# Arthur151/ROMP

Measured on NVIDIA H100. Metric: frames/sec 512x512 ROMP-HRNet32 (whole hot path), higher is better.
Workload: dtype bf16

## Files before the change

### romp_b200/csrc/conv_block_tc.cu

```cuda
#include "conv_tc.cuh"
#include "tc_device.cuh"

namespace b200romp {

namespace {

constexpr int kBlkThreads = 384;
constexpr int kRowB = 128;
constexpr int kHaloW = 12, kHaloH = 20;
constexpr int kTapBytes = 64 * kRowB;
constexpr int kWBytes = 9 * kTapBytes;
constexpr int kStagePayload = kHaloH * kHaloW * kRowB;
constexpr int kStageBytes = (282 * kRowB + 1023) / 1024 * 1024;
constexpr int kMidBytes = 256 * kRowB;
constexpr int kSmemBytes = 2 * kWBytes + kStageBytes + kMidBytes + 1024  + 1024 ;
static_assert(kSmemBytes <= 227 * 1024, "fused block does not fit shared memory");

template <bool FOLD>
__device__ __forceinline__ constexpr bool blk_skip(int tap, int k) {
  return FOLD && ((tap % 3 == 0 && k < 2) || (tap % 3 == 2 && k >= 2));
}

__device__ __forceinline__ void consumers_bar_sync() { asm volatile("bar.sync 1, 256;" ::: "memory"); }

__device__ __forceinline__ uint32_t ld_shared_b32(uint32_t addr) {
  uint32_t v;
  asm volatile("ld.shared.b32 %0, [%1];" : "=r"(v) : "r"(addr));
  return v;
}
__device__ __forceinline__ void st_shared_b32(uint32_t addr, uint32_t v) {
  asm volatile("st.shared.b32 [%0], %1;" ::"r"(addr), "r"(v) : "memory");
}
template <typename T>
__device__ __forceinline__ T opaque(T v) {
  uint64_t u = (uint64_t)v;
  asm volatile("mov.b64 %0, %0;" : "+l"(u));
  return (T)u;
}
__device__ __forceinline__ uint32_t pack_bf16x2(float a, float b) {
  const __nv_bfloat162 v = __floats2bfloat162_rn(a, b);
  return *reinterpret_cast<const uint32_t*>(&v);
}

}

template <bool FOLD>
__global__ void __launch_bounds__(kBlkThreads, 1)
conv_block_tc_kernel(const __grid_constant__ CUtensorMap tmap, const ConvParams p, const uint8_t* __restrict__ w1pack,
                     const uint8_t* __restrict__ w2pack, const float* __restrict__ bias1, int tiles_x, int tiles_y, int num_tiles) {
  extern __shared__ uint8_t smem_raw[];
  uint8_t* smem = reinterpret_cast<uint8_t*>((reinterpret_cast<uintptr_t>(smem_raw) + 1023) & ~(uintptr_t)1023);
  uint8_t* sW1 = smem;
  uint8_t* sW2 = smem + kWBytes;
  uint8_t* sA = smem + 2 * kWBytes;
  uint8_t* sMid = sA + kStageBytes;
  uint64_t* full = reinterpret_cast<uint64_t*>(sMid + kMidBytes);
  uint64_t* empty = full + 1;
  uint64_t* w_full = full + 2;

  const int warp = threadIdx.x >> 5;
  if (threadIdx.x == 0) {
    mbar_init(full, 1);
    mbar_init(empty, 256);
    mbar_init(w_full, 1);
    fence_barrier_init();
  }
  __syncthreads();
  pdl_trigger();
  const int per_frame = tiles_x * tiles_y;

  if (warp == 0) {
    if (elect_one()) {
      mbar_arrive_expect_tx(w_full, 2 * kWBytes);
      for (int t = 0; t < 9; ++t) {
        bulk_copy_g2s(sW1 + t * kTapBytes, w1pack + (size_t)t * kTapBytes, kTapBytes, w_full);
        bulk_copy_g2s(sW2 + t * kTapBytes, w2pack + (size_t)t * kTapBytes, kTapBytes, w_full);
      }
      pdl_wait();
      const uint64_t pol = l2_policy_stream();
      uint32_t phase = 0;
      for (int tile = blockIdx.x; tile < num_tiles; tile += gridDim.x, phase ^= 1) {
        const int n = tile / per_frame, rem = tile % per_frame;
        const int y0 = (rem / tiles_x) * 16, x0 = (rem % tiles_x) * 8;
        mbar_wait(empty, phase ^ 1);
        mbar_arrive_expect_tx(full, kStagePayload);
        tma_load_4d(sA, &tmap, full, 0, x0 - 2, y0 - 2, n, pol);
      }
    }
  } else if (warp >= 4) {
    const int g = (warp >> 2) - 1, t = threadIdx.x & 127, w = t >> 5, l = t & 31;
    pdl_wait();
    mbar_wait(w_full, 0);
    const int cl = 2 * (l & 3);
    uint32_t phase = 0;
    for (int tile = blockIdx.x; tile < num_tiles; tile += gridDim.x, phase ^= 1) {
      const uint32_t w1_base = opaque(smem_u32(sW1)), w2_base = opaque(smem_u32(sW2)), a_base = opaque(smem_u32(sA)),
                     mid_base = opaque(smem_u32(sMid));
      const float* b1p = opaque(bias1);
      const float* b2p = opaque(p.bias);
      const int n = tile / per_frame, rem = tile % per_frame;
      const int y0 = (rem / tiles_x) * 16, x0 = (rem % tiles_x) * 8;
      mbar_wait(full, phase);

      float acc[2][32];
#pragma unroll
      for (int h = 0; h < 2; ++h)
#pragma unroll
        for (int j = 0; j < 32; ++j) acc[h][j] = 0.f;
      uint32_t scale_d = 0;
      wgmma_fence();
#pragma unroll
      for (int tap = 0; tap < 9; ++tap) {
        const uint32_t a_tap = a_base + (uint32_t)((128 * g + (tap / 3) * kHaloW + tap % 3) * kRowB);
        const uint32_t b_tap = w1_base + (uint32_t)(tap * kTapBytes);
#pragma unroll
        for (int k = 0; k < 4; ++k) {
          if (blk_skip<FOLD>(tap, k)) continue;
          const uint64_t bdesc = make_smem_desc(b_tap + k * 32, 8 * kRowB, kSw128);
          wgmma_n64(acc[0], make_smem_desc(a_tap + k * 32, 8 * kRowB, kSw128), bdesc, scale_d, false);
          wgmma_n64(acc[1], make_smem_desc(a_tap + 64 * kRowB + k * 32, 8 * kRowB, kSw128), bdesc, scale_d, false);
          scale_d = 1;
        }
      }
      wgmma_commit();
      uint32_t rv[2][8];
#pragma unroll
      for (int e = 0; e < 2; ++e) {
        const int hr = (8 * g + 2 * w + e + 2) * kHaloW + (l >> 2) + 2;
#pragma unroll
        for (int j = 0; j < 8; ++j) rv[e][j] = ld_shared_b32(a_base + hr * kRowB + ((j ^ (hr & 7)) << 4) + 2 * cl);
      }
      wgmma_wait<0>();
      mbar_arrive(empty);

      consumers_bar_sync();
#pragma unroll
      for (int h = 0; h < 2; ++h) {
#pragma unroll
        for (int e = 0; e < 2; ++e) {
          const int m = 64 * (2 * g + h) + 16 * w + (l >> 2) + 8 * e;
          const int my = m / kHaloW, mx = m % kHaloW;
          const bool inside = my < 18 && mx < 10 && (unsigned)(y0 - 1 + my) < (unsigned)p.Hout && (unsigned)(x0 - 1 + mx) < (unsigned)p.Wout;
          const uint32_t row = mid_base + m * kRowB;
#pragma unroll
          for (int j = 0; j < 8; ++j) {
            const int c = 8 * j + cl;
            float a = fmaxf(acc[h][4 * j + 2 * e] + __ldg(b1p + c), 0.f);
            float b = fmaxf(acc[h][4 * j + 2 * e + 1] + __ldg(b1p + c + 1), 0.f);
            if (!inside) a = b = 0.f;
            st_shared_b32(row + ((j ^ (m & 7)) << 4) + 2 * cl, pack_bf16x2(a, b));
          }
        }
      }
      fence_proxy_async();
      consumers_bar_sync();

      float acc2[32];
#pragma unroll
      for (int j = 0; j < 32; ++j) acc2[j] = 0.f;
      scale_d = 0;
      wgmma_fence();
#pragma unroll
      for (int tap = 0; tap < 9; ++tap) {
        const uint32_t a_tap = mid_base + (uint32_t)(((8 * g + tap / 3) * kHaloW + tap % 3) * kRowB);
        const uint32_t b_tap = w2_base + (uint32_t)(tap * kTapBytes);
#pragma unroll
        for (int k = 0; k < 4; ++k) {
          if (blk_skip<FOLD>(tap, k)) continue;
          wgmma_n64(acc2, make_smem_desc(a_tap + k * 32, kHaloW * kRowB, kSw128), make_smem_desc(b_tap + k * 32, 8 * kRowB, kSw128),
                    scale_d, false);
          scale_d = 1;
        }
      }
      wgmma_commit();
      wgmma_wait<0>();

      __nv_bfloat16* out = reinterpret_cast<__nv_bfloat16*>(p.out);
#pragma unroll
      for (int e = 0; e < 2; ++e) {
        const size_t pix = ((size_t)n * p.Hout + y0 + 8 * g + 2 * w + e) * p.Wout + x0 + (l >> 2);
        __nv_bfloat162* o = reinterpret_cast<__nv_bfloat162*>(out + pix * p.out_C + p.out_c_off + cl);
#pragma unroll
        for (int j = 0; j < 8; ++j) {
          const int c = 8 * j + cl;
          float a = acc2[4 * j + 2 * e] + __ldg(b2p + c), b = acc2[4 * j + 2 * e + 1] + __ldg(b2p + c + 1);
          const float2 r = res_pair(rv[e][j]);
          a += r.x; b += r.y;
          o[4 * j] = __floats2bfloat162_rn(fmaxf(a, 0.f), fmaxf(b, 0.f));
        }
      }
    }
  }
}

bool tc_block_supported(const ConvParams& p) {
  if (p.in_dtype != B200ROMP_BF16 || p.out_dtype != B200ROMP_BF16 || p.res_dtype != B200ROMP_BF16) return false;
  if (p.cin != 64 || p.cout != 64 || p.up != 1 || p.out_nchw || p.pow_channel >= 0 || p.input_norm || !p.relu) return false;
  if (p.Hin != p.Hout || p.Win != p.Wout || p.Hout % 16 != 0 || p.Wout % 8 != 0) return false;
  if (p.in_C % 8 != 0 || p.in_c_off % 8 != 0 || p.out_C % 8 != 0 || p.out_c_off % 8 != 0) return false;
  if (p.res != p.in || p.res_C != p.in_C || p.res_c_off != p.in_c_off || p.res_broadcast) return false;
  return (reinterpret_cast<uintptr_t>(p.in) & 15) == 0;
}

int tc_block_prepare(const ConvParams& p, const float* w1_oihw, const float* b1, const float* w2_oihw, int sm_count,
                     TcConvPlan* plan, std::vector<void*>* allocs) {
  PFN_encodeTiled encode = tc_get_encode();
  if (!encode) {
    set_error("conv_block_tc: cuTensorMapEncodeTiled is unavailable");
    return B200ROMP_ECUDA;
  }
  plan->kind = 60;
  plan->eb = 2;
  plan->cin = plan->cout = plan->nt = 64;
  plan->grid_x = sm_count;
  plan->grid_y = 1;
  plan->stages = 1;
  plan->smem_bytes = kSmemBytes;
  int rc = tc_pack_weights(w1_oihw, 64, 64, 9, 64, &plan->d_wpack, allocs, kRowB, 2);
  if (rc) return rc;
  rc = tc_pack_weights(w2_oihw, 64, 64, 9, 64, &plan->d_wpack2, allocs, kRowB, 2);
  if (rc) return rc;
  void* db1 = nullptr;
  B2R_CUDA_OK(cudaMalloc(&db1, 64 * sizeof(float)));
  allocs->push_back(db1);
  B2R_CUDA_OK(cudaMemcpy(db1, b1, 64 * sizeof(float), cudaMemcpyHostToDevice));
  plan->d_bias1 = static_cast<const float*>(db1);
  CUtensorMap tm;
  const cuuint64_t gdim[4] = {64, (cuuint64_t)p.Win, (cuuint64_t)p.Hin, (cuuint64_t)p.B};
  const cuuint64_t gstr[3] = {(cuuint64_t)p.in_C * 2, (cuuint64_t)p.Win * p.in_C * 2, (cuuint64_t)p.Hin * p.Win * p.in_C * 2};
  const cuuint32_t box[4] = {64, kHaloW, kHaloH, 1};
  const cuuint32_t estr[4] = {1, 1, 1, 1};
  void* base = const_cast<uint8_t*>(static_cast<const uint8_t*>(p.in) + (size_t)p.in_c_off * 2);
  CUresult cr = encode(&tm, CU_TENSOR_MAP_DATA_TYPE_BFLOAT16, 4, base, gdim, gstr, box, estr, CU_TENSOR_MAP_INTERLEAVE_NONE,
                       CU_TENSOR_MAP_SWIZZLE_128B, CU_TENSOR_MAP_L2_PROMOTION_L2_128B, CU_TENSOR_MAP_FLOAT_OOB_FILL_NONE);
  if (cr != CUDA_SUCCESS) {
    set_error("conv_block_tc: cuTensorMapEncodeTiled failed with %d", (int)cr);
    return B200ROMP_ECUDA;
  }
  memcpy(plan->tmap_in, &tm, sizeof(tm));
  B2R_CUDA_OK(cudaFuncSetAttribute(conv_block_tc_kernel<false>, cudaFuncAttributeMaxDynamicSharedMemorySize, kSmemBytes));
  B2R_CUDA_OK(cudaFuncSetAttribute(conv_block_tc_kernel<true>, cudaFuncAttributeMaxDynamicSharedMemorySize, kSmemBytes));
  return B200ROMP_OK;
}

int tc_block_launch(const TcConvPlan& plan, const ConvParams& p, cudaStream_t stream) {
  CUtensorMap tm;
  memcpy(&tm, plan.tmap_in, sizeof(tm));
  const int tiles_x = p.Wout / 8, tiles_y = p.Hout / 16;
  const int num_tiles = tiles_x * tiles_y * p.B;
  const dim3 grid(std::min(plan.grid_x, num_tiles));
  auto kern = plan.fold ? conv_block_tc_kernel<true> : conv_block_tc_kernel<false>;
  B2R_CUDA_OK(tc_launch(kern, grid, kBlkThreads, plan.smem_bytes, stream, tm, p, reinterpret_cast<const uint8_t*>(plan.d_wpack),
                        reinterpret_cast<const uint8_t*>(plan.d_wpack2), plan.d_bias1, tiles_x, tiles_y, num_tiles));
  return B200ROMP_OK;
}

}
```

Baseline: 3221.

## Ping-pong two consumer warpgroups over double-buffered tiles in fused residual block

Restructures the fused conv-conv residual block so each consumer warpgroup owns a whole tile in its own double-buffered smem slot, and the two warpgroups alternate issuing their wgmma phases through 'issued' mbarriers. The conv1 output is written back into the input slot instead of a separate mid buffer. Producer and consumer register budgets are rebalanced with setmaxnreg, and bias values are hoisted into registers once per CTA. The aim is to overlap one warpgroup's epilogue with the other's tensor-core work and to take the TMA load off the critical path. The cost is higher register pressure (two conv1 accumulator sets per thread) and more complex barrier phase logic.

Result: faster. 3274 (median of 6 runs) (+1.6%).

```diff
diff --git a/romp_b200/csrc/conv_block_tc.cu b/romp_b200/csrc/conv_block_tc.cu
--- a/romp_b200/csrc/conv_block_tc.cu
+++ b/romp_b200/csrc/conv_block_tc.cu
@@ -10,18 +10,26 @@
 constexpr int kHaloW = 12, kHaloH = 20;
 constexpr int kTapBytes = 64 * kRowB;
 constexpr int kWBytes = 9 * kTapBytes;
-constexpr int kStagePayload = kHaloH * kHaloW * kRowB;
-constexpr int kStageBytes = (282 * kRowB + 1023) / 1024 * 1024;
-constexpr int kMidBytes = 256 * kRowB;
-constexpr int kSmemBytes = 2 * kWBytes + kStageBytes + kMidBytes + 1024  + 1024 ;
+constexpr int kSlotBytes = kHaloH * kHaloW * kRowB;
+constexpr int kMidRows = (kHaloH - 2) * kHaloW - 2;
+constexpr int kConv1Rows = 256;
+constexpr int kPadBytes = (kConv1Rows + 2 * kHaloW + 2) * kRowB - kSlotBytes;
+constexpr int kSmemBytes = 2 * kWBytes + 2 * kSlotBytes + kPadBytes + 64  + 1024 ;
+static_assert(kSlotBytes % 1024 == 0, "a slot must start on the 1024 B anchor of the 128 B swizzle");
+static_assert(kMidRows - 1 + 2 * kHaloW + 2 < kHaloH * kHaloW, "conv1 rows conv2 reads must stay inside their slot");
 static_assert(kSmemBytes <= 227 * 1024, "fused block does not fit shared memory");
+constexpr int kProducerRegs = 40, kConsumerRegs = 232;
+static_assert(128 * kProducerRegs + 256 * kConsumerRegs <= 65536, "register file");
 
 template <bool FOLD>
 __device__ __forceinline__ constexpr bool blk_skip(int tap, int k) {
   return FOLD && ((tap % 3 == 0 && k < 2) || (tap % 3 == 2 && k >= 2));
 }
 
-__device__ __forceinline__ void consumers_bar_sync() { asm volatile("bar.sync 1, 256;" ::: "memory"); }
+template <int N>
+__device__ __forceinline__ void setmaxnreg_dec() { asm volatile("setmaxnreg.dec.sync.aligned.u32 %0;" ::"n"(N)); }
+template <int N>
+__device__ __forceinline__ void setmaxnreg_inc() { asm volatile("setmaxnreg.inc.sync.aligned.u32 %0;" ::"n"(N)); }
 
 __device__ __forceinline__ uint32_t ld_shared_b32(uint32_t addr) {
   uint32_t v;
@@ -31,15 +39,116 @@
 __device__ __forceinline__ void st_shared_b32(uint32_t addr, uint32_t v) {
   asm volatile("st.shared.b32 [%0], %1;" ::"r"(addr), "r"(v) : "memory");
 }
-template <typename T>
-__device__ __forceinline__ T opaque(T v) {
-  uint64_t u = (uint64_t)v;
-  asm volatile("mov.b64 %0, %0;" : "+l"(u));
-  return (T)u;
+__device__ __forceinline__ uint32_t opaque(uint32_t v) {
+  asm volatile("mov.b32 %0, %0;" : "+r"(v));
+  return v;
 }
 __device__ __forceinline__ uint32_t pack_bf16x2(float a, float b) {
   const __nv_bfloat162 v = __floats2bfloat162_rn(a, b);
   return *reinterpret_cast<const uint32_t*>(&v);
+}
+
+template <bool FOLD>
+__device__ __forceinline__ void blk_conv1(float (&acc)[2][32], uint32_t slot, uint32_t w1_base, int q) {
+#pragma unroll
+  for (int h = 0; h < 2; ++h)
+#pragma unroll
+    for (int j = 0; j < 32; ++j) acc[h][j] = 0.f;
+  uint32_t scale_d = 0;
+  wgmma_fence();
+#pragma unroll
+  for (int tap = 0; tap < 9; ++tap) {
+    const uint32_t a_tap = slot + (uint32_t)((128 * q + (tap / 3) * kHaloW + tap % 3) * kRowB);
+    const uint32_t b_tap = w1_base + (uint32_t)(tap * kTapBytes);
+#pragma unroll
+    for (int k = 0; k < 4; ++k) {
+      if (blk_skip<FOLD>(tap, k)) continue;
+      const uint64_t bdesc = make_smem_desc(b_tap + k * 32, 8 * kRowB, kSw128);
+      wgmma_n64(acc[0], make_smem_desc(a_tap + k * 32, 8 * kRowB, kSw128), bdesc, scale_d, false);
+      wgmma_n64(acc[1], make_smem_desc(a_tap + 64 * kRowB + k * 32, 8 * kRowB, kSw128), bdesc, scale_d, false);
+      scale_d = 1;
+    }
+  }
+  wgmma_commit();
+}
+
+__device__ __forceinline__ void blk_load_residual(uint32_t (&rv)[2][2][8], uint32_t slot, int w, int l) {
+  const int cl = 2 * (l & 3);
+#pragma unroll
+  for (int h = 0; h < 2; ++h)
+#pragma unroll
+    for (int e = 0; e < 2; ++e) {
+      const int hr = (8 * h + 2 * w + e + 2) * kHaloW + (l >> 2) + 2;
+#pragma unroll
+      for (int j = 0; j < 8; ++j) rv[h][e][j] = ld_shared_b32(slot + hr * kRowB + ((j ^ (hr & 7)) << 4) + 2 * cl);
+    }
+}
+
+__device__ __forceinline__ void blk_mid_store(const float (&acc)[2][32], uint32_t slot, int q, const float2 (&b1)[8], const ConvParams& p,
+                                              int y0, int x0, int w, int l) {
+  const int cl = 2 * (l & 3);
+#pragma unroll
+  for (int h = 0; h < 2; ++h) {
+#pragma unroll
+    for (int e = 0; e < 2; ++e) {
+      const int m = 64 * (2 * q + h) + 16 * w + (l >> 2) + 8 * e;
+      if (m >= kMidRows) continue;
+      const int my = m / kHaloW, mx = m % kHaloW;
+      const bool inside = mx < 10 && (unsigned)(y0 - 1 + my) < (unsigned)p.Hout && (unsigned)(x0 - 1 + mx) < (unsigned)p.Wout;
+      const uint32_t row = slot + m * kRowB;
+#pragma unroll
+      for (int j = 0; j < 8; ++j) {
+        float a = fmaxf(acc[h][4 * j + 2 * e] + b1[j].x, 0.f);
+        float b = fmaxf(acc[h][4 * j + 2 * e + 1] + b1[j].y, 0.f);
+        if (!inside) a = b = 0.f;
+        st_shared_b32(row + ((j ^ (m & 7)) << 4) + 2 * cl, pack_bf16x2(a, b));
+      }
+    }
+  }
+}
+
+template <bool FOLD>
+__device__ __forceinline__ void blk_conv2(float (&acc2)[2][32], uint32_t slot, uint32_t w2_base) {
+#pragma unroll
+  for (int h = 0; h < 2; ++h)
+#pragma unroll
+    for (int j = 0; j < 32; ++j) acc2[h][j] = 0.f;
+  uint32_t scale_d = 0;
+  wgmma_fence();
+#pragma unroll
+  for (int tap = 0; tap < 9; ++tap) {
+    const uint32_t a_tap = slot + (uint32_t)(((tap / 3) * kHaloW + tap % 3) * kRowB);
+    const uint32_t b_tap = w2_base + (uint32_t)(tap * kTapBytes);
+#pragma unroll
+    for (int k = 0; k < 4; ++k) {
+      if (blk_skip<FOLD>(tap, k)) continue;
+      const uint64_t bdesc = make_smem_desc(b_tap + k * 32, 8 * kRowB, kSw128);
+      wgmma_n64(acc2[0], make_smem_desc(a_tap + k * 32, kHaloW * kRowB, kSw128), bdesc, scale_d, false);
+      wgmma_n64(acc2[1], make_smem_desc(a_tap + 8 * kHaloW * kRowB + k * 32, kHaloW * kRowB, kSw128), bdesc, scale_d, false);
+      scale_d = 1;
+    }
+  }
+  wgmma_commit();
+}
+
+__device__ __forceinline__ void blk_out_epilogue(const float (&acc2)[2][32], const uint32_t (&rv)[2][2][8], const float2 (&b2)[8],
+                                                 const ConvParams& p, int n, int y0, int x0, int w, int l) {
+  const int cl = 2 * (l & 3);
+  __nv_bfloat16* out = reinterpret_cast<__nv_bfloat16*>(p.out);
+#pragma unroll
+  for (int h = 0; h < 2; ++h)
+#pragma unroll
+    for (int e = 0; e < 2; ++e) {
+      const size_t pix = ((size_t)n * p.Hout + y0 + 8 * h + 2 * w + e) * p.Wout + x0 + (l >> 2);
+      __nv_bfloat162* o = reinterpret_cast<__nv_bfloat162*>(out + pix * p.out_C + p.out_c_off + cl);
+#pragma unroll
+      for (int j = 0; j < 8; ++j) {
+        float a = acc2[h][4 * j + 2 * e] + b2[j].x, b = acc2[h][4 * j + 2 * e + 1] + b2[j].y;
+        const float2 r = res_pair(rv[h][e][j]);
+        a += r.x; b += r.y;
+        o[4 * j] = __floats2bfloat162_rn(fmaxf(a, 0.f), fmaxf(b, 0.f));
+      }
+    }
 }
 
 }
@@ -53,24 +162,34 @@
   uint8_t* sW1 = smem;
   uint8_t* sW2 = smem + kWBytes;
   uint8_t* sA = smem + 2 * kWBytes;
-  uint8_t* sMid = sA + kStageBytes;
-  uint64_t* full = reinterpret_cast<uint64_t*>(sMid + kMidBytes);
-  uint64_t* empty = full + 1;
-  uint64_t* w_full = full + 2;
+  uint64_t* full = reinterpret_cast<uint64_t*>(sA + 2 * kSlotBytes + kPadBytes);
+  uint64_t* empty = full + 2;
+  uint64_t* issued = full + 4;
+  uint64_t* w_full = full + 6;
 
   const int warp = threadIdx.x >> 5;
   if (threadIdx.x == 0) {
-    mbar_init(full, 1);
-    mbar_init(empty, 256);
+    for (int s = 0; s < 2; ++s) {
+      mbar_init(&full[s], 1);
+      mbar_init(&empty[s], 128);
+      mbar_init(&issued[s], 128);
+    }
     mbar_init(w_full, 1);
     fence_barrier_init();
   }
   __syncthreads();
   pdl_trigger();
   const int per_frame = tiles_x * tiles_y;
-
-  if (warp == 0) {
-    if (elect_one()) {
+  auto origin = [&](int tile, int& n, int& y0, int& x0) {
+    n = tile / per_frame;
+    const int rem = tile % per_frame;
+    y0 = (rem / tiles_x) * 16;
+    x0 = (rem % tiles_x) * 8;
+  };
+
+  if (warp < 4) {
+    setmaxnreg_dec<kProducerRegs>();
+    if (warp == 0 && elect_one()) {
       mbar_arrive_expect_tx(w_full, 2 * kWBytes);
       for (int t = 0; t < 9; ++t) {
         bulk_copy_g2s(sW1 + t * kTapBytes, w1pack + (size_t)t * kTapBytes, kTapBytes, w_full);
@@ -78,117 +197,69 @@
       }
       pdl_wait();
       const uint64_t pol = l2_policy_stream();
-      uint32_t phase = 0;
-      for (int tile = blockIdx.x; tile < num_tiles; tile += gridDim.x, phase ^= 1) {
-        const int n = tile / per_frame, rem = tile % per_frame;
-        const int y0 = (rem / tiles_x) * 16, x0 = (rem % tiles_x) * 8;
-        mbar_wait(empty, phase ^ 1);
-        mbar_arrive_expect_tx(full, kStagePayload);
-        tma_load_4d(sA, &tmap, full, 0, x0 - 2, y0 - 2, n, pol);
+      int i = 0;
+      for (int tile = blockIdx.x; tile < num_tiles; tile += gridDim.x, ++i) {
+        int n, y0, x0;
+        origin(tile, n, y0, x0);
+        const int s = i & 1;
+        mbar_wait(&empty[s], ((i >> 1) & 1) ^ 1);
+        mbar_arrive_expect_tx(&full[s], kSlotBytes);
+        tma_load_4d(sA + s * kSlotBytes, &tmap, &full[s], 0, x0 - 2, y0 - 2, n, pol);
       }
     }
-  } else if (warp >= 4) {
+  } else {
+    setmaxnreg_inc<kConsumerRegs>();
     const int g = (warp >> 2) - 1, t = threadIdx.x & 127, w = t >> 5, l = t & 31;
     pdl_wait();
     mbar_wait(w_full, 0);
-    const int cl = 2 * (l & 3);
-    uint32_t phase = 0;
-    for (int tile = blockIdx.x; tile < num_tiles; tile += gridDim.x, phase ^= 1) {
-      const uint32_t w1_base = opaque(smem_u32(sW1)), w2_base = opaque(smem_u32(sW2)), a_base = opaque(smem_u32(sA)),
-                     mid_base = opaque(smem_u32(sMid));
-      const float* b1p = opaque(bias1);
-      const float* b2p = opaque(p.bias);
-      const int n = tile / per_frame, rem = tile % per_frame;
-      const int y0 = (rem / tiles_x) * 16, x0 = (rem % tiles_x) * 8;
-      mbar_wait(full, phase);
-
-      float acc[2][32];
-#pragma unroll
-      for (int h = 0; h < 2; ++h)
-#pragma unroll
-        for (int j = 0; j < 32; ++j) acc[h][j] = 0.f;
-      uint32_t scale_d = 0;
-      wgmma_fence();
-#pragma unroll
-      for (int tap = 0; tap < 9; ++tap) {
-        const uint32_t a_tap = a_base + (uint32_t)((128 * g + (tap / 3) * kHaloW + tap % 3) * kRowB);
-        const uint32_t b_tap = w1_base + (uint32_t)(tap * kTapBytes);
-#pragma unroll
-        for (int k = 0; k < 4; ++k) {
-          if (blk_skip<FOLD>(tap, k)) continue;
-          const uint64_t bdesc = make_smem_desc(b_tap + k * 32, 8 * kRowB, kSw128);
-          wgmma_n64(acc[0], make_smem_desc(a_tap + k * 32, 8 * kRowB, kSw128), bdesc, scale_d, false);
-          wgmma_n64(acc[1], make_smem_desc(a_tap + 64 * kRowB + k * 32, 8 * kRowB, kSw128), bdesc, scale_d, false);
-          scale_d = 1;
-        }
-      }
-      wgmma_commit();
-      uint32_t rv[2][8];
-#pragma unroll
-      for (int e = 0; e < 2; ++e) {
-        const int hr = (8 * g + 2 * w + e + 2) * kHaloW + (l >> 2) + 2;
-#pragma unroll
-        for (int j = 0; j < 8; ++j) rv[e][j] = ld_shared_b32(a_base + hr * kRowB + ((j ^ (hr & 7)) << 4) + 2 * cl);
-      }
+    const uint32_t w1_base = smem_u32(sW1), w2_base = smem_u32(sW2), slot_base = smem_u32(sA) + g * kSlotBytes;
+    float2 b1[8], b2[8];
+#pragma unroll
+    for (int j = 0; j < 8; ++j) {
+      b1[j] = __ldg(reinterpret_cast<const float2*>(bias1 + 8 * j + 2 * (l & 3)));
+      b2[j] = __ldg(reinterpret_cast<const float2*>(p.bias + 8 * j + 2 * (l & 3)));
+    }
+    const int cta_tiles = (num_tiles - blockIdx.x + gridDim.x - 1) / gridDim.x;
+    const int wg1_phases = 2 * (cta_tiles / 2);
+    int phase_k = 0;
+    auto wait_turn = [&]() {
+      if (g == 1) mbar_wait(&issued[0], phase_k & 1);
+      else if (phase_k > 0 && phase_k - 1 < wg1_phases) mbar_wait(&issued[1], (phase_k - 1) & 1);
+    };
+    auto pass_turn = [&]() {
+      mbar_arrive(&issued[g]);
+      ++phase_k;
+    };
+    uint32_t parity = 0;
+    for (int i = g; i < cta_tiles; i += 2, parity ^= 1) {
+      int n, y0, x0;
+      origin(blockIdx.x + i * gridDim.x, n, y0, x0);
+      const uint32_t slot = opaque(slot_base);
+      mbar_wait(&full[g], parity);
+
+      float acc1[2][2][32];
+      wait_turn();
+      blk_conv1<FOLD>(acc1[0], slot, opaque(w1_base), 0);
+      blk_conv1<FOLD>(acc1[1], slot, opaque(w1_base), 1);
+      pass_turn();
+      uint32_t rv[2][2][8];
+      blk_load_residual(rv, slot, w, l);
+      wgmma_wait<1>();
+      wg_bar_sync(1 + g);
+      blk_mid_store(acc1[0], slot, 0, b1, p, y0, x0, w, l);
       wgmma_wait<0>();
-      mbar_arrive(empty);
-
-      consumers_bar_sync();
-#pragma unroll
-      for (int h = 0; h < 2; ++h) {
-#pragma unroll
-        for (int e = 0; e < 2; ++e) {
-          const int m = 64 * (2 * g + h) + 16 * w + (l >> 2) + 8 * e;
-          const int my = m / kHaloW, mx = m % kHaloW;
-          const bool inside = my < 18 && mx < 10 && (unsigned)(y0 - 1 + my) < (unsigned)p.Hout && (unsigned)(x0 - 1 + mx) < (unsigned)p.Wout;
-          const uint32_t row = mid_base + m * kRowB;
-#pragma unroll
-          for (int j = 0; j < 8; ++j) {
-            const int c = 8 * j + cl;
-            float a = fmaxf(acc[h][4 * j + 2 * e] + __ldg(b1p + c), 0.f);
-            float b = fmaxf(acc[h][4 * j + 2 * e + 1] + __ldg(b1p + c + 1), 0.f);
-            if (!inside) a = b = 0.f;
-            st_shared_b32(row + ((j ^ (m & 7)) << 4) + 2 * cl, pack_bf16x2(a, b));
-          }
-        }
-      }
+      wg_bar_sync(1 + g);
+      blk_mid_store(acc1[1], slot, 1, b1, p, y0, x0, w, l);
       fence_proxy_async();
-      consumers_bar_sync();
-
-      float acc2[32];
-#pragma unroll
-      for (int j = 0; j < 32; ++j) acc2[j] = 0.f;
-      scale_d = 0;
-      wgmma_fence();
-#pragma unroll
-      for (int tap = 0; tap < 9; ++tap) {
-        const uint32_t a_tap = mid_base + (uint32_t)(((8 * g + tap / 3) * kHaloW + tap % 3) * kRowB);
-        const uint32_t b_tap = w2_base + (uint32_t)(tap * kTapBytes);
-#pragma unroll
-        for (int k = 0; k < 4; ++k) {
-          if (blk_skip<FOLD>(tap, k)) continue;
-          wgmma_n64(acc2, make_smem_desc(a_tap + k * 32, kHaloW * kRowB, kSw128), make_smem_desc(b_tap + k * 32, 8 * kRowB, kSw128),
-                    scale_d, false);
-          scale_d = 1;
-        }
-      }
-      wgmma_commit();
+      wg_bar_sync(1 + g);
+
+      float acc2[2][32];
+      wait_turn();
+      blk_conv2<FOLD>(acc2, slot, opaque(w2_base));
+      pass_turn();
       wgmma_wait<0>();
-
-      __nv_bfloat16* out = reinterpret_cast<__nv_bfloat16*>(p.out);
-#pragma unroll
-      for (int e = 0; e < 2; ++e) {
-        const size_t pix = ((size_t)n * p.Hout + y0 + 8 * g + 2 * w + e) * p.Wout + x0 + (l >> 2);
-        __nv_bfloat162* o = reinterpret_cast<__nv_bfloat162*>(out + pix * p.out_C + p.out_c_off + cl);
-#pragma unroll
-        for (int j = 0; j < 8; ++j) {
-          const int c = 8 * j + cl;
-          float a = acc2[4 * j + 2 * e] + __ldg(b2p + c), b = acc2[4 * j + 2 * e + 1] + __ldg(b2p + c + 1);
-          const float2 r = res_pair(rv[e][j]);
-          a += r.x; b += r.y;
-          o[4 * j] = __floats2bfloat162_rn(fmaxf(a, 0.f), fmaxf(b, 0.f));
-        }
-      }
+      mbar_arrive(&empty[g]);
+      blk_out_epilogue(acc2, rv, b2, p, n, y0, x0, w, l);
     }
   }
 }
```
